# sosp2021/Reth

Measured on AMD Instinct MI355X. Metric: env-steps/sec + learner updates/sec, Ape-X DQN Pong, 1/2/4/8 MI355X, higher is better.
Workload: dtype f32

## Files before the change

### reth_amd/csrc/fc.hip

```cpp
#include <type_traits>
#include <utility>

#include "common.hpp"
#include "fc_rows.hpp"

namespace rth {

using f32x4 = __attribute__((ext_vector_type(4))) float;

constexpr int kFcTm = 64, kFcTn = 128, kFcThreads = 256;
__device__ __forceinline__ float fc_relu(float v) { return v < 0.0f ? 0.0f : v; }
constexpr int kFcBUnits = 8 * 3 * 64;

template <int... I, class F>
__device__ __forceinline__ void static_for(std::integer_sequence<int, I...>, F &&f) {
  (f(std::integral_constant<int, I>{}), ...);
}

template <int PF>
__global__ __launch_bounds__(kFcThreads) void k_fc_x9(const float *__restrict__ x, int64_t ldx, int M,
                                                      const float *__restrict__ w, int N, int K, int splits,
                                                      const float *__restrict__ bias, int relu,
                                                      float *__restrict__ out) {
  __shared__ uint4 bl[2][kFcBUnits];
  const int tid = threadIdx.x, lane = tid & 63, g = lane >> 4, r = lane & 15;
  const int wave = __builtin_amdgcn_readfirstlane(tid >> 6);
  const int tiles_n = N / kFcTn;
  const int tile = (int)blockIdx.x / splits, split = (int)blockIdx.x % splits;
  const int m0 = (tile / tiles_n) * kFcTm, n0 = (tile % tiles_n) * kFcTn;
  const int chunks = K / 32;
  const int c0 = chunks * split / splits, c1 = chunks * (split + 1) / splits;
  const int wn = tid & 127, wh = tid >> 7;
  const float *wrow = w + (int64_t)(n0 + wn) * K + 16 * wh;
  const float *xrow = x + (int64_t)(m0 + 16 * wave + r) * ldx + 8 * g;
  constexpr int NR = PF + 1;
  f32x4 wv[NR][4], xv[NR][2];
  auto load = [&](int c, f32x4 (&wl)[4], f32x4 (&xl)[2]) __attribute__((always_inline)) {
#pragma unroll
    for (int j = 0; j < 4; ++j) wl[j] = *reinterpret_cast<const f32x4 *>(wrow + 32 * c + 4 * j);
#pragma unroll
    for (int j = 0; j < 2; ++j) xl[j] = *reinterpret_cast<const f32x4 *>(xrow + 32 * c + 4 * j);
  };
  auto stage = [&](const f32x4 (&wl)[4], uint4 *buf) __attribute__((always_inline)) {
    const int nb = wn >> 4, rr = wn & 15;
#pragma unroll
    for (int h = 0; h < 2; ++h) {
      const float v[8] = {wl[2 * h][0], wl[2 * h][1], wl[2 * h][2], wl[2 * h][3],
                          wl[2 * h + 1][0], wl[2 * h + 1][1], wl[2 * h + 1][2], wl[2 * h + 1][3]};
      bf16x8 tr[3];
      split3_pk8(v, tr);
#pragma unroll
      for (int t = 0; t < 3; ++t) buf[(nb * 3 + t) * 64 + rr + 16 * (2 * wh + h)] = __builtin_bit_cast(uint4, tr[t]);
    }
  };
  f32x4 acc[8];
#pragma unroll
  for (int nb = 0; nb < 8; ++nb) acc[nb] = f32x4{0.f, 0.f, 0.f, 0.f};
  auto compute = [&](const f32x4 (&xl)[2], const uint4 *buf) __attribute__((always_inline)) {
    const float v[8] = {xl[0][0], xl[0][1], xl[0][2], xl[0][3], xl[1][0], xl[1][1], xl[1][2], xl[1][3]};
    bf16x8 af[3];
    split3_pk8(v, af);
#pragma unroll
    for (int nb = 0; nb < 8; ++nb) {
      bf16x8 b[3];
#pragma unroll
      for (int t = 0; t < 3; ++t) b[t] = __builtin_bit_cast(bf16x8, buf[(nb * 3 + t) * 64 + lane]);
      f32x4 a = acc[nb];
      a = __builtin_amdgcn_mfma_f32_16x16x32_bf16(af[2], b[2], a, 0, 0, 0);
      a = __builtin_amdgcn_mfma_f32_16x16x32_bf16(af[2], b[1], a, 0, 0, 0);
      a = __builtin_amdgcn_mfma_f32_16x16x32_bf16(af[1], b[2], a, 0, 0, 0);
      a = __builtin_amdgcn_mfma_f32_16x16x32_bf16(af[2], b[0], a, 0, 0, 0);
      a = __builtin_amdgcn_mfma_f32_16x16x32_bf16(af[1], b[1], a, 0, 0, 0);
      a = __builtin_amdgcn_mfma_f32_16x16x32_bf16(af[0], b[2], a, 0, 0, 0);
      a = __builtin_amdgcn_mfma_f32_16x16x32_bf16(af[1], b[0], a, 0, 0, 0);
      a = __builtin_amdgcn_mfma_f32_16x16x32_bf16(af[0], b[1], a, 0, 0, 0);
      a = __builtin_amdgcn_mfma_f32_16x16x32_bf16(af[0], b[0], a, 0, 0, 0);
      acc[nb] = a;
    }
  };
  auto iter = [&](int c, auto ic) __attribute__((always_inline)) {
    constexpr int i = decltype(ic)::value;
    constexpr int pr = i % NR, pl = i & 1;
    compute(xv[pr], bl[pl]);
    stage(wv[(i + 1) % NR], bl[pl ^ 1]);
    const int cn = c + NR < c1 ? c + NR : c1 - 1;
    load(cn, wv[pr], xv[pr]);
    __syncthreads();
  };
#pragma unroll
  for (int q = 0; q < NR; ++q) load(c0 + q < c1 ? c0 + q : c1 - 1, wv[q], xv[q]);
  stage(wv[0], bl[0]);
  __syncthreads();
  int c = c0;
  constexpr int U = 2 * NR;
  for (; c + U <= c1; c += U)
    static_for(std::make_integer_sequence<int, U>{}, [&](auto ic) __attribute__((always_inline)) {
      iter(c + decltype(ic)::value, ic);
    });
  static_for(std::make_integer_sequence<int, U>{}, [&](auto ic) __attribute__((always_inline)) {
    if (c + decltype(ic)::value < c1) iter(c + decltype(ic)::value, ic);
  });
  const int mrow = m0 + 16 * wave + 4 * g;
  if (splits == 1) {
#pragma unroll
    for (int nb = 0; nb < 8; ++nb) {
      const int n = n0 + 16 * nb + r;
      const float bn = bias ? bias[n] : 0.0f;
#pragma unroll
      for (int i = 0; i < 4; ++i) {
        const float v = radd(acc[nb][i], bn);
        out[(int64_t)(mrow + i) * N + n] = relu ? fc_relu(v) : v;
      }
    }
  } else {
    float *part = out + (int64_t)split * M * N;
#pragma unroll
    for (int nb = 0; nb < 8; ++nb)
#pragma unroll
      for (int i = 0; i < 4; ++i) part[(int64_t)(mrow + i) * N + n0 + 16 * nb + r] = acc[nb][i];
  }
}

constexpr int kFbTile = 128;
__host__ __device__ constexpr int fc_ta(int k) { return (int)((0x221210100ull >> (4 * (8 - k))) & 15); }
__host__ __device__ constexpr int fc_tb(int k) { return (int)((0x212012010ull >> (4 * (8 - k))) & 15); }
static_assert(fc_ta(0) == 2 && fc_tb(0) == 2 && fc_ta(3) == 2 && fc_tb(3) == 0 && fc_ta(5) == 0 && fc_tb(5) == 2 &&
                  fc_ta(8) == 0 && fc_tb(8) == 0 && fc_ta(6) == 1 && fc_tb(6) == 0,
              "term order");
constexpr int kFbUnits = 8 * 3 * 64;
template <int WAVES, int PF>
__global__ __launch_bounds__(WAVES * 64) void k_fc_x9t(const float *__restrict__ x, int64_t ldx, int M,
                                                      const float *__restrict__ w, int N, int K, int splits,
                                                      const float *__restrict__ bias, int relu,
                                                      float *__restrict__ out) {
  constexpr int T = WAVES * 64, WN = WAVES / 2, NB = 8 / WN;
  constexpr int RH = 2 * 2 * kFbTile / T;
  constexpr int NR = PF + 1;
  static_assert(WAVES == 4 || WAVES == 8, "4 or 8 waves");
  __shared__ uint4 sl[2][2][kFbUnits];
  const int tid = threadIdx.x, lane = tid & 63, g = lane >> 4, r = lane & 15;
  const int wave = __builtin_amdgcn_readfirstlane(tid >> 6), wm = wave & 1, wn = wave >> 1;
  const int tiles_n = N / kFbTile;
  const int tile = (int)blockIdx.x / splits, split = (int)blockIdx.x % splits;
  const int m0 = (tile / tiles_n) * kFbTile, n0 = (tile % tiles_n) * kFbTile;
  const int chunks = K / 32;
  const int c0 = chunks * split / splits, c1 = chunks * (split + 1) / splits;
  const float *src[RH];
#pragma unroll
  for (int j = 0; j < RH; ++j) {
    const int u = tid + j * T, op = u >> 8, rr = u & 127, h = (u >> 7) & 1;
    src[j] = op == 0 ? x + (int64_t)(m0 + rr) * ldx + 16 * h : w + (int64_t)(n0 + rr) * K + 16 * h;
  }
  f32x4 ring[NR][RH][4];
  auto load = [&](int c, f32x4 (&v)[RH][4]) __attribute__((always_inline)) {
#pragma unroll
    for (int j = 0; j < RH; ++j)
#pragma unroll
      for (int q = 0; q < 4; ++q) v[j][q] = *reinterpret_cast<const f32x4 *>(src[j] + 32 * c + 4 * q);
  };
  auto stage = [&](const f32x4 (&v)[RH][4], uint4 (*buf)[kFbUnits]) __attribute__((always_inline)) {
#pragma unroll
    for (int j = 0; j < RH; ++j) {
      const int u = tid + j * T, op = u >> 8, rr = u & 127, h = (u >> 7) & 1;
      const int blk = rr >> 4, rw = rr & 15;
#pragma unroll
      for (int hh = 0; hh < 2; ++hh) {
        const float vv[8] = {v[j][2 * hh][0], v[j][2 * hh][1], v[j][2 * hh][2], v[j][2 * hh][3],
                             v[j][2 * hh + 1][0], v[j][2 * hh + 1][1], v[j][2 * hh + 1][2], v[j][2 * hh + 1][3]};
        bf16x8 tr[3];
        split3_pk8(vv, tr);
#pragma unroll
        for (int t = 0; t < 3; ++t) buf[op][(blk * 3 + t) * 64 + rw + 16 * (2 * h + hh)] = __builtin_bit_cast(uint4, tr[t]);
      }
    }
  };
  f32x4 acc[4][NB];
#pragma unroll
  for (int mb = 0; mb < 4; ++mb)
#pragma unroll
    for (int nb = 0; nb < NB; ++nb) acc[mb][nb] = f32x4{0.f, 0.f, 0.f, 0.f};
  auto compute = [&](uint4 (*buf)[kFbUnits]) __attribute__((always_inline)) {
    bf16x8 af[4][3], bfr[NB][3];
#pragma unroll
    for (int mb = 0; mb < 4; ++mb)
#pragma unroll
      for (int t = 0; t < 3; ++t) af[mb][t] = __builtin_bit_cast(bf16x8, buf[0][((4 * wm + mb) * 3 + t) * 64 + lane]);
#pragma unroll
    for (int nb = 0; nb < NB; ++nb)
#pragma unroll
      for (int t = 0; t < 3; ++t)
        bfr[nb][t] = __builtin_bit_cast(bf16x8, buf[1][((NB * wn + nb) * 3 + t) * 64 + lane]);
#pragma unroll
    for (int k = 0; k < 9; ++k)
#pragma unroll
      for (int mb = 0; mb < 4; ++mb)
#pragma unroll
        for (int nb = 0; nb < NB; ++nb)
          acc[mb][nb] = __builtin_amdgcn_mfma_f32_16x16x32_bf16(af[mb][fc_ta(k)], bfr[nb][fc_tb(k)], acc[mb][nb], 0, 0, 0);
  };
  auto clampc = [&](int c) { return c < c1 ? c : c1 - 1; };
#pragma unroll
  for (int q = 0; q < NR; ++q) load(clampc(c0 + q), ring[q]);
  stage(ring[0], sl[0]);
  load(clampc(c0 + NR), ring[0]);
  __syncthreads();
  auto iter = [&](int i, auto ic) __attribute__((always_inline)) {
    constexpr int s = decltype(ic)::value;
    compute(sl[s & 1]);
    stage(ring[(s + 1) % NR], sl[(s + 1) & 1]);
    load(clampc(c0 + i + 1 + NR), ring[(s + 1) % NR]);
    __syncthreads();
  };
  const int n_it = c1 - c0;
  constexpr int U = 2 * NR;
  int i = 0;
  for (; i + U <= n_it; i += U)
    static_for(std::make_integer_sequence<int, U>{}, [&](auto ic) __attribute__((always_inline)) {
      iter(i + decltype(ic)::value, ic);
    });
  static_for(std::make_integer_sequence<int, U>{}, [&](auto ic) __attribute__((always_inline)) {
    if (i + decltype(ic)::value < n_it) iter(i + decltype(ic)::value, ic);
  });
  float *dst = splits == 1 ? out : out + (int64_t)split * M * N;
#pragma unroll
  for (int mb = 0; mb < 4; ++mb)
#pragma unroll
    for (int nb = 0; nb < NB; ++nb) {
      const int n = n0 + 16 * (NB * wn + nb) + r;
      const float bn = splits == 1 && bias ? bias[n] : 0.0f;
#pragma unroll
      for (int e = 0; e < 4; ++e) {
        const int m = m0 + 64 * wm + 16 * mb + 4 * g + e;
        float v = acc[mb][nb][e];
        if (splits == 1) {
          v = radd(v, bn);
          v = relu ? fc_relu(v) : v;
        }
        dst[(int64_t)m * N + n] = v;
      }
    }
}

constexpr int kFfTm = 64, kFfTn = 128, kFfThreads = 256;
template <int NST>
__global__ __launch_bounds__(kFfThreads) void k_fc_f32(const float *__restrict__ x, int64_t ldx, int M,
                                                       const float *__restrict__ w, int N, int K, int splits,
                                                       const float *__restrict__ bias, int relu,
                                                       float *__restrict__ out) {
  const int tid = threadIdx.x, lane = tid & 63, g = lane >> 4, r = lane & 15;
  const int wave = __builtin_amdgcn_readfirstlane(tid >> 6), wm = wave & 1, wn = wave >> 1;
  const int split = (int)blockIdx.x % splits, tile = (int)blockIdx.x / splits;
  const int tiles_n = N / kFfTn;
  const int m0 = (tile / tiles_n) * kFfTm + 32 * wm, n0 = (tile % tiles_n) * kFfTn + 64 * wn;
  const int chunks = K / 32;
  const int c0 = chunks * split / splits, c1 = chunks * (split + 1) / splits;
  const __amdgpu_buffer_rsrc_t xs = __builtin_amdgcn_make_buffer_rsrc(const_cast<float *>(x), 0,
                                                                      (int)(((int64_t)(M - 1) * ldx + K) * 4), 0x00020000);
  const __amdgpu_buffer_rsrc_t ws = __builtin_amdgcn_make_buffer_rsrc(const_cast<float *>(w), 0,
                                                                      (int)((int64_t)N * K * 4), 0x00020000);
  uint32_t xo[2], wo[4];
#pragma unroll
  for (int mb = 0; mb < 2; ++mb) {
    const int row = m0 + 16 * mb + r;
    xo[mb] = (uint32_t)(((int64_t)(row < M ? row : M - 1) * ldx + 8 * g) * 4);
  }
#pragma unroll
  for (int nb = 0; nb < 4; ++nb) wo[nb] = (uint32_t)(((int64_t)(n0 + 16 * nb + r) * K + 8 * g) * 4);
  f32x4 xa[NST][2][2], wb[NST][4][2];
  auto ld = [](__amdgpu_buffer_rsrc_t rs, uint32_t vo, int so) {
    return __builtin_bit_cast(f32x4, __builtin_amdgcn_raw_buffer_load_b128(rs, vo, so, 0));
  };
  auto load = [&](int c, f32x4 (&a)[2][2], f32x4 (&b)[4][2]) __attribute__((always_inline)) {
    const int so = c * 128;
#pragma unroll
    for (int nb = 0; nb < 4; ++nb)
#pragma unroll
      for (int h = 0; h < 2; ++h) b[nb][h] = ld(ws, wo[nb] + 16 * h, so);
#pragma unroll
    for (int mb = 0; mb < 2; ++mb)
#pragma unroll
      for (int h = 0; h < 2; ++h) a[mb][h] = ld(xs, xo[mb] + 16 * h, so);
  };
  f32x4 acc[2][4];
#pragma unroll
  for (int mb = 0; mb < 2; ++mb)
#pragma unroll
    for (int nb = 0; nb < 4; ++nb) acc[mb][nb] = f32x4{0.f, 0.f, 0.f, 0.f};
  auto compute = [&](const f32x4 (&a)[2][2], const f32x4 (&b)[4][2]) __attribute__((always_inline)) {
#pragma unroll
    for (int h = 0; h < 2; ++h)
#pragma unroll
      for (int t = 0; t < 4; ++t)
#pragma unroll
        for (int mb = 0; mb < 2; ++mb)
#pragma unroll
          for (int nb = 0; nb < 4; ++nb)
            acc[mb][nb] = __builtin_amdgcn_mfma_f32_16x16x4f32(a[mb][h][t], b[nb][h][t], acc[mb][nb], 0, 0, 0);
  };
#pragma unroll
  for (int s = 0; s < NST; ++s) load(c0 + s < c1 ? c0 + s : c1 - 1, xa[s], wb[s]);
  auto iter = [&](int c, auto is) __attribute__((always_inline)) {
    constexpr int s = decltype(is)::value;
    compute(xa[s], wb[s]);
    const int cn = c + NST < c1 ? c + NST : c1 - 1;
    load(cn, xa[s], wb[s]);
    __builtin_amdgcn_sched_barrier(0);
  };
  int c = c0;
  for (; c + NST <= c1; c += NST)
    static_for(std::make_integer_sequence<int, NST>{}, [&](auto is) __attribute__((always_inline)) {
      iter(c + decltype(is)::value, is);
    });
  static_for(std::make_integer_sequence<int, NST>{}, [&](auto is) __attribute__((always_inline)) {
    if (c + decltype(is)::value < c1) compute(xa[decltype(is)::value], wb[decltype(is)::value]);
  });
  float *dst = splits == 1 ? out : out + (int64_t)split * M * N;
#pragma unroll
  for (int mb = 0; mb < 2; ++mb)
#pragma unroll
    for (int i = 0; i < 4; ++i) {
      const int m = m0 + 16 * mb + 4 * g + i;
      if (m < M) {
#pragma unroll
        for (int nb = 0; nb < 4; ++nb) {
          const int n = n0 + 16 * nb + r;
          float v = acc[mb][nb][i];
          if (splits == 1) {
            v = radd(v, bias ? bias[n] : 0.0f);
            v = relu ? fc_relu(v) : v;
          }
          dst[(int64_t)m * N + n] = v;
        }
      }
    }
}

template <int MAXS>
__device__ __forceinline__ void fc_reduce_wg(int blk, const float *__restrict__ part, int splits, int64_t MN, int N,
                                             const float *__restrict__ bias, int relu, float *__restrict__ y,
                                             int64_t ldy) {
  const int64_t e4 = ((int64_t)blk * 256 + threadIdx.x) * 4;
  if (e4 >= MN) return;
  f32x4 v[MAXS];
#pragma unroll
  for (int k = 0; k < MAXS; ++k) v[k] = *reinterpret_cast<const f32x4 *>(part + (int64_t)(k < splits ? k : splits - 1) * MN + e4);
  f32x4 s = v[0];
#pragma unroll
  for (int k = 1; k < MAXS; ++k)
    if (k < splits) {
#pragma unroll
      for (int j = 0; j < 4; ++j) s[j] = radd(s[j], v[k][j]);
    }
  const int64_t m = e4 / N;
  const int n = (int)(e4 - m * N);
  f32x4 o;
#pragma unroll
  for (int j = 0; j < 4; ++j) {
    const float t = radd(s[j], bias ? bias[n + j] : 0.0f);
    o[j] = relu ? fc_relu(t) : t;
  }
  *reinterpret_cast<f32x4 *>(y + m * ldy + n) = o;
}

template <int MAXS>
__global__ __launch_bounds__(256) void k_fc_reduce(const float *__restrict__ part, int splits, int64_t MN, int N,
                                                   const float *__restrict__ bias, int relu, float *__restrict__ y,
                                                   int64_t ldy) {
  fc_reduce_wg<MAXS>((int)blockIdx.x, part, splits, MN, N, bias, relu, y, ldy);
}

constexpr int kRhRows = 4, kRhMaxN = 512;
template <int MAXS, int MAXA1>
__global__ __launch_bounds__(256) __attribute__((amdgpu_waves_per_eu(1, 3))) void k_fc_reduce_heads(const float *__restrict__ part, int splits, int M, int N,
                                                         const float *__restrict__ b1, int A,
                                                         const float *__restrict__ wa2, const float *__restrict__ wv2,
                                                         const float *__restrict__ ba2, const float *__restrict__ bv2,
                                                         float *__restrict__ heads, float *__restrict__ h1_out) {
  __shared__ f32x4 hs[kRhRows * kRhMaxN / 4];
  const int r0 = (int)blockIdx.x * kRhRows, N4 = N / 4;
  const int64_t MN = (int64_t)M * N;
  constexpr int PER = kRhRows * kRhMaxN / 4 / 256;
  f32x4 v[PER][MAXS];
  const __amdgpu_buffer_rsrc_t pr =
      __builtin_amdgcn_make_buffer_rsrc(const_cast<float *>(part), 0, (int)(splits * MN * 4), 0x00020000);
#pragma unroll
  for (int u = 0; u < PER; ++u) {
    const int i = (int)threadIdx.x + 256 * u, rr = i / N4;
    const int row = r0 + rr < M ? r0 + rr : M - 1;
    const uint32_t off = (uint32_t)(((int64_t)row * N + 4 * (i - rr * N4)) * 4);
#pragma unroll
    for (int k = 0; k < MAXS; ++k)
      v[u][k] = __builtin_bit_cast(
          f32x4, __builtin_amdgcn_raw_buffer_load_b128(pr, off, (int)((k < splits ? k : splits - 1) * MN * 4), 0));
  }
  __builtin_amdgcn_sched_barrier(0);
#pragma unroll
  for (int u = 0; u < PER; ++u) {
    const int i = (int)threadIdx.x + 256 * u, rr = i / N4, c = 4 * (i - rr * N4);
    if (i >= kRhRows * N4) break;
    f32x4 sum = v[u][0];
#pragma unroll
    for (int k = 1; k < MAXS; ++k)
      if (k < splits) {
#pragma unroll
        for (int j = 0; j < 4; ++j) sum[j] = radd(sum[j], v[u][k][j]);
      }
    f32x4 o;
#pragma unroll
    for (int j = 0; j < 4; ++j) o[j] = fc_relu(radd(sum[j], b1[c + j]));
    hs[i] = o;
    if (h1_out && r0 + rr < M) *reinterpret_cast<f32x4 *>(h1_out + (int64_t)(r0 + rr) * N + c) = o;
  }
  __syncthreads();
  if (threadIdx.x >= 16 * kRhRows) return;
  const int l = threadIdx.x & 15, rr = threadIdx.x >> 4;
  const int H = N / 2, cq = H / 64, A1 = A + 1;
  const f32x4 *ha = hs + rr * N4 + l * cq, *hv = hs + rr * N4 + H / 4 + l * cq;
  float acc[MAXA1];
#pragma unroll
  for (int a = 0; a < MAXA1; ++a) acc[a] = 0.0f;
#pragma unroll 1
  for (int k = 0; k < cq; ++k) {
    const f32x4 xa = ha[k], xv = hv[k];
    float4 w[MAXA1];
#pragma unroll
    for (int a = 0; a < MAXA1; ++a) {
      const int ac = a < A1 ? a : A;
      w[a] = reinterpret_cast<const float4 *>(ac < A ? wa2 + (int64_t)ac * H : wv2)[l * cq + k];
    }
#pragma unroll
    for (int a = 0; a < MAXA1; ++a)
      if (a < A1) {
        const f32x4 x = a < A ? xa : xv;
        const float4 ww = w[a];
        acc[a] = radd(radd(radd(radd(acc[a], rmul(x[0], ww.x)), rmul(x[1], ww.y)), rmul(x[2], ww.z)), rmul(x[3], ww.w));
      }
  }
#pragma unroll
  for (int a = 0; a < MAXA1; ++a)
#pragma unroll
    for (int o = 1; o < 16; o <<= 1) acc[a] = radd(acc[a], __shfl_xor(acc[a], o, 64));
  if (l == 0 && r0 + rr < M) {
    float *out = heads + (int64_t)(r0 + rr) * A1;
#pragma unroll
    for (int a = 0; a < MAXA1; ++a)
      if (a <= A) out[a] = radd(acc[a], a < A ? ba2[a] : bv2[0]);
  }
}

static_assert(kLrThreads == 256, "k_fc_reduce_rows runs k_linear_relu_rows' workgroups at 256 lanes");
template <int MAXS>
__global__ __launch_bounds__(256) void k_fc_reduce_rows(const float *__restrict__ part, int splits, int64_t MN, int N,
                                                        const float *__restrict__ bias, float *__restrict__ y,
                                                        int64_t ldy, int nred, const float *__restrict__ x,
                                                        int64_t ldx, int64_t r0, int64_t n_max,
                                                        const int64_t *__restrict__ n_dev,
                                                        const float *__restrict__ w, int K) {
  if ((int)blockIdx.x < nred)
    fc_reduce_wg<MAXS>((int)blockIdx.x, part, splits, MN, N, bias, 1, y, ldy);
  else
    linear_relu_rows_wg((int)blockIdx.x - nred, x, ldx, r0, n_max, n_dev, w, bias, K, N, y, ldy);
}

static const void *fc_reduce_fn(int splits, bool rows) {
  if (rows)
    return splits <= 4    ? reinterpret_cast<const void *>(&k_fc_reduce_rows<4>)
           : splits <= 8  ? reinterpret_cast<const void *>(&k_fc_reduce_rows<8>)
           : splits <= 16 ? reinterpret_cast<const void *>(&k_fc_reduce_rows<16>)
                          : reinterpret_cast<const void *>(&k_fc_reduce_rows<32>);
  return splits <= 4    ? reinterpret_cast<const void *>(&k_fc_reduce<4>)
         : splits <= 8  ? reinterpret_cast<const void *>(&k_fc_reduce<8>)
         : splits <= 16 ? reinterpret_cast<const void *>(&k_fc_reduce<16>)
                        : reinterpret_cast<const void *>(&k_fc_reduce<32>);
}
static int launch_fc_reduce(const float *part, int splits, int64_t MN, int N, const float *bias, int relu, float *y,
                            int64_t ldy, hipStream_t s) {
  RTH_REQUIRE(splits >= 1 && splits <= 32, "fc reduce: %d splits", splits);
  void *args[] = {&part, &splits, &MN, &N, &bias, &relu, &y, &ldy};
  RTH_HIP(hipLaunchKernel(fc_reduce_fn(splits, false), dim3((unsigned)((MN / 4 + 255) / 256)), dim3(256), args, 0, s));
  return RTH_OK;
}

static int fc_splits(int M, int N, int K) {
  const int tiles = (M / kFcTm) * (N / kFcTn), chunks = K / 32;
  int s = (256 + tiles - 1) / tiles;
  s = s < 1 ? 1 : (s > 32 ? 32 : s);
  return s < chunks ? s : chunks;
}

struct FcPlan {
  int big, splits;
};
constexpr int kFcMaxSplits = 16;
static FcPlan fc_plan(int M, int N, int K) {
  if (M % kFbTile || N % kFbTile) return FcPlan{0, fc_splits(M, N, K)};
  const int tiles = (M / kFbTile) * (N / kFbTile), chunks = K / 32;
  int s = (256 + tiles - 1) / tiles;
  s = s > kFcMaxSplits ? kFcMaxSplits : (s < 1 ? 1 : s);
  return FcPlan{1, s < chunks ? s : chunks};
}

static void fc_x9_launch(const FcPlan &p, const float *x, int64_t ldx, int M, const float *w, int N, int K,
                         const float *bias, int relu, float *out, hipStream_t s) {
  if (!p.big) {
    const int tiles = (M / kFcTm) * (N / kFcTn);
    hipLaunchKernelGGL(k_fc_x9<2>, dim3((unsigned)(tiles * p.splits)), dim3(kFcThreads), 0, s, x, ldx, M, w, N, K,
                       p.splits, bias, relu, out);
    return;
  }
  const dim3 grid((unsigned)((M / kFbTile) * (N / kFbTile) * p.splits));
  hipLaunchKernelGGL((k_fc_x9t<8, 1>), grid, dim3(512), 0, s, x, ldx, M, w, N, K, p.splits, bias, relu, out);
}

static int fcf_splits(int M, int N, int K) {
  const int tiles = ((M + kFfTm - 1) / kFfTm) * (N / kFfTn), chunks = K / 32;
  int s = 8;
  while (s > 1 && tiles * s > 512) s /= 2;
  return s < chunks ? s : chunks;
}

constexpr int kFwTn = 64, kFwThreads = 256;
constexpr int kFwAUnits = 8 * 3 * 64, kFwUnits = kFwAUnits + 4 * 3 * 64;
template <bool AT, int MB>
__device__ __forceinline__ void fc_bwd_tile(uint4 (*sl)[kFwUnits], const float *__restrict__ a, int64_t lda,
                                            const float *__restrict__ b, int64_t ldb, float *__restrict__ out,
                                            int64_t ldo, int m0, int n0, int c0, int c1) {
  constexpr int TM = 32 * MB, T = kFwThreads, NR = 2;
  constexpr int ATASKS = AT ? 4 * TM : 2 * TM, AJ = (ATASKS + T - 1) / T;
  const int tid = threadIdx.x, lane = tid & 63, g = lane >> 4, r = lane & 15;
  const int wave = __builtin_amdgcn_readfirstlane(tid >> 6), wm = wave & 1, wn = wave >> 1;
  const float *asrc[AJ];
#pragma unroll
  for (int j = 0; j < AJ; ++j) {
    const int u = tid + j * T, rr = u % TM, h = u / TM;
    asrc[j] = AT ? a + (int64_t)(8 * h) * lda + m0 + rr : a + (int64_t)(m0 + rr) * lda + 16 * h;
  }
  const float *bsrc = b + (int64_t)(8 * (tid >> 6)) * ldb + n0 + (tid & 63);
  f32x4 ra4[NR][AJ][4];
  float ra1[NR][AJ][8];
  float rb[NR][8];
  auto load = [&](int c, int s) __attribute__((always_inline)) {
#pragma unroll
    for (int j = 0; j < AJ; ++j)
      if (tid + j * T < ATASKS) {
        if constexpr (AT) {
#pragma unroll
          for (int q = 0; q < 8; ++q) ra1[s][j][q] = asrc[j][(int64_t)(32 * c + q) * lda];
        } else {
#pragma unroll
          for (int q = 0; q < 4; ++q) ra4[s][j][q] = *reinterpret_cast<const f32x4 *>(asrc[j] + 32 * c + 4 * q);
        }
      }
#pragma unroll
    for (int q = 0; q < 8; ++q) rb[s][q] = bsrc[(int64_t)(32 * c + q) * ldb];
  };
  auto put = [&](const float (&v)[8], uint4 *dst) __attribute__((always_inline)) {
    bf16x8 tr[3];
    split3_pk8(v, tr);
#pragma unroll
    for (int t = 0; t < 3; ++t) dst[t * 64] = __builtin_bit_cast(uint4, tr[t]);
  };
  auto stage = [&](int s, uint4 *buf) __attribute__((always_inline)) {
#pragma unroll
    for (int j = 0; j < AJ; ++j)
      if (tid + j * T < ATASKS) {
        const int u = tid + j * T, rr = u % TM, h = u / TM;
        uint4 *blk = buf + (rr >> 4) * 3 * 64 + (rr & 15);
        if constexpr (AT) {
          put(ra1[s][j], blk + 16 * h);
        } else {
#pragma unroll
          for (int hh = 0; hh < 2; ++hh) {
            const f32x4 lo = ra4[s][j][2 * hh], hi = ra4[s][j][2 * hh + 1];
            const float v[8] = {lo[0], lo[1], lo[2], lo[3], hi[0], hi[1], hi[2], hi[3]};
            put(v, blk + 16 * (2 * h + hh));
          }
        }
      }
    const int col = tid & 63;
    put(rb[s], buf + kFwAUnits + (col >> 4) * 3 * 64 + (col & 15) + 16 * (tid >> 6));
  };
  f32x4 acc[MB][2], lo[MB][2];
#pragma unroll
  for (int mb = 0; mb < MB; ++mb)
#pragma unroll
    for (int nb = 0; nb < 2; ++nb) acc[mb][nb] = lo[mb][nb] = f32x4{0.f, 0.f, 0.f, 0.f};
  auto compute = [&](const uint4 *buf) __attribute__((always_inline)) {
    bf16x8 af[MB][3], bfr[2][3];
#pragma unroll
    for (int mb = 0; mb < MB; ++mb)
#pragma unroll
      for (int t = 0; t < 3; ++t) af[mb][t] = __builtin_bit_cast(bf16x8, buf[((MB * wm + mb) * 3 + t) * 64 + lane]);
#pragma unroll
    for (int nb = 0; nb < 2; ++nb)
#pragma unroll
      for (int t = 0; t < 3; ++t)
        bfr[nb][t] = __builtin_bit_cast(bf16x8, buf[kFwAUnits + ((2 * wn + nb) * 3 + t) * 64 + lane]);
    static_assert(fc_ta(8) == 0 && fc_tb(8) == 0, "the leading term is the last");
#pragma unroll
    for (int k = 0; k < 9; ++k)
#pragma unroll
      for (int mb = 0; mb < MB; ++mb)
#pragma unroll
        for (int nb = 0; nb < 2; ++nb) {
          f32x4 &d = k < 8 ? lo[mb][nb] : acc[mb][nb];
          d = __builtin_amdgcn_mfma_f32_16x16x32_bf16(af[mb][fc_ta(k)], bfr[nb][fc_tb(k)], d, 0, 0, 0);
        }
  };
  auto clampc = [&](int c) { return c < c1 ? c : c1 - 1; };
  load(c0, 0);
  load(clampc(c0 + 1), 1);
  stage(0, sl[0]);
  load(clampc(c0 + 2), 0);
  __syncthreads();
  auto iter = [&](int i, auto is) __attribute__((always_inline)) {
    constexpr int s = decltype(is)::value;
    compute(sl[s]);
    stage(s ^ 1, sl[s ^ 1]);
    load(clampc(c0 + i + 3), s ^ 1);
    __syncthreads();
  };
  const int n_it = c1 - c0;
  int i = 0;
  for (; i + 2 <= n_it; i += 2) {
    iter(i, std::integral_constant<int, 0>{});
    iter(i + 1, std::integral_constant<int, 1>{});
  }
  if (i < n_it) iter(i, std::integral_constant<int, 0>{});
#pragma unroll
  for (int mb = 0; mb < MB; ++mb)
#pragma unroll
    for (int nb = 0; nb < 2; ++nb)
#pragma unroll
      for (int e = 0; e < 4; ++e)
        out[(int64_t)(m0 + 16 * (MB * wm + mb) + 4 * g + e) * ldo + n0 + 16 * (2 * wn + nb) + r] =
            radd(acc[mb][nb][e], lo[mb][nb][e]);
}

template <int MBD>
__global__ __launch_bounds__(kFwThreads) void k_fc_bwd(const float *__restrict__ gy, int64_t ldg,
                                                       const float *__restrict__ x, int64_t ldx,
                                                       const float *__restrict__ w, int B, int N, int K,
                                                       float *__restrict__ gx_out, float *__restrict__ gw_out,
                                                       int nblk_d, int sd, int sw) {
  __shared__ uint4 sl[2][kFwUnits];
  const int tiles_k = K / kFwTn;
  int blk = (int)blockIdx.x;
  if (blk < nblk_d) {
    const int tile = blk / sd, split = blk % sd, chunks = N / 32;
    fc_bwd_tile<false, MBD>(sl, gy, ldg, w, K, gx_out + (int64_t)split * B * K, K, (tile / tiles_k) * 32 * MBD,
                            (tile % tiles_k) * kFwTn, chunks * split / sd, chunks * (split + 1) / sd);
  } else {
    blk -= nblk_d;
    const int tile = blk / sw, split = blk % sw, chunks = B / 32;
    fc_bwd_tile<true, 4>(sl, gy, ldg, x, ldx, gw_out + (int64_t)split * N * K, K, (tile / tiles_k) * 128,
                         (tile % tiles_k) * kFwTn, chunks * split / sw, chunks * (split + 1) / sw);
  }
}

template <int MAXS>
__global__ __launch_bounds__(256) void k_fc_bwd_reduce(const float *__restrict__ pd, int sd, int64_t MNd,
                                                       float *__restrict__ gx, int nred_d,
                                                       const float *__restrict__ pw, int sw, int64_t MNw,
                                                       float *__restrict__ gw, int K) {
  if ((int)blockIdx.x < nred_d)
    fc_reduce_wg<MAXS>((int)blockIdx.x, pd, sd, MNd, K, nullptr, 0, gx, K);
  else
    fc_reduce_wg<MAXS>((int)blockIdx.x - nred_d, pw, sw, MNw, K, nullptr, 0, gw, K);
}

constexpr int kFwMaxSplits = 8;
struct FcBwdPlan {
  int mbd, tiles_d, sd, tiles_w, sw;
};
static FcBwdPlan fc_bwd_plan(int B, int N, int K) {
  auto splits = [](int tiles, int chunks) {
    int s = 1;
    while (2 * s * tiles <= 256 && 4 * s <= chunks && 2 * s <= kFwMaxSplits) s *= 2;
    return s;
  };
  FcBwdPlan p;
  p.mbd = B % 128 == 0 ? 4 : 2;
  p.tiles_d = (B / (32 * p.mbd)) * (K / kFwTn);
  p.sd = splits(p.tiles_d, N / 32);
  p.tiles_w = (N / 128) * (K / kFwTn);
  p.sw = splits(p.tiles_w, B / 32);
  return p;
}

}

using namespace rth;

extern "C" {

int rth_fc_bwd_supported(int64_t B, int64_t N, int64_t K) {
  return B > 0 && B % 64 == 0 && N > 0 && N % 128 == 0 && K > 0 && K % kFwTn == 0 && B * K < (1ll << 31) &&
                 N * K < (1ll << 31) && B * N < (1ll << 31)
             ? 1
             : 0;
}

int64_t rth_fc_bwd_workspace(int64_t B, int64_t N, int64_t K) {
  if (!rth_fc_bwd_supported(B, N, K)) return 0;
  const FcBwdPlan p = fc_bwd_plan((int)B, (int)N, (int)K);
  return (p.sd > 1 ? (int64_t)p.sd * B * K * 4 : 0) + (p.sw > 1 ? (int64_t)p.sw * N * K * 4 : 0);
}

int rth_fc_bwd(const float *gy, int64_t ldg, const float *x, int64_t ldx, const float *w, int64_t B, int64_t N,
               int64_t K, float *gx, float *gw, void *workspace, void *stream) {
  RTH_REQUIRE(gy && (gx || gw), "rth_fc_bwd: NULL gy, or neither gradient asked for");
  RTH_REQUIRE((!gx || w) && (!gw || x), "rth_fc_bwd: NULL operand of a gradient asked for");
  RTH_REQUIRE(rth_fc_bwd_supported(B, N, K), "rth_fc_bwd: shape %lld x %lld x %lld not built (B %% 64, N %% 128, K %% 64)",
              (long long)B, (long long)N, (long long)K);
  RTH_REQUIRE(ldg >= N && ldg % 4 == 0 && (!gw || (ldx >= K && ldx % 4 == 0)) && (B - 1) * ldg + N < (1ll << 31) &&
                  (!gw || (B - 1) * ldx + K < (1ll << 31)),
              "rth_fc_bwd: row strides %lld, %lld", (long long)ldg, (long long)ldx);
  RTH_REQUIRE(((reinterpret_cast<uintptr_t>(gy) | reinterpret_cast<uintptr_t>(x) | reinterpret_cast<uintptr_t>(w) |
                reinterpret_cast<uintptr_t>(gx) | reinterpret_cast<uintptr_t>(gw)) &
               15) == 0,
              "rth_fc_bwd: misaligned buffer");
  const FcBwdPlan p = fc_bwd_plan((int)B, (int)N, (int)K);
  const int sd = gx ? p.sd : 1, sw = gw ? p.sw : 1;
  RTH_REQUIRE((sd == 1 && sw == 1) || (workspace && (reinterpret_cast<uintptr_t>(workspace) & 15) == 0),
              "rth_fc_bwd: %d / %d splits need the workspace (rth_fc_bwd_workspace)", sd, sw);
  hipStream_t s = as_stream(stream);
  float *pd = static_cast<float *>(workspace);
  float *pw = pd ? pd + (p.sd > 1 ? (int64_t)p.sd * B * K : 0) : nullptr;
  float *od = sd > 1 ? pd : gx, *ow = sw > 1 ? pw : gw;
  const int nblk_d = gx ? p.tiles_d * sd : 0, nblk_w = gw ? p.tiles_w * sw : 0;
  const dim3 grid((unsigned)(nblk_d + nblk_w));
  if (p.mbd == 4)
    hipLaunchKernelGGL(k_fc_bwd<4>, grid, dim3(kFwThreads), 0, s, gy, ldg, x, ldx, w, (int)B, (int)N, (int)K, od, ow,
                       nblk_d, sd, sw);
  else
    hipLaunchKernelGGL(k_fc_bwd<2>, grid, dim3(kFwThreads), 0, s, gy, ldg, x, ldx, w, (int)B, (int)N, (int)K, od, ow,
                       nblk_d, sd, sw);
  RTH_LAUNCHED();
  if (sd > 1 || sw > 1) {
    const int64_t MNd = B * K, MNw = N * K;
    const int nred_d = sd > 1 ? (int)((MNd / 4 + 255) / 256) : 0, nred_w = sw > 1 ? (int)((MNw / 4 + 255) / 256) : 0;
    const dim3 rgrid((unsigned)(nred_d + nred_w));
    if (sd <= 4 && sw <= 4)
      hipLaunchKernelGGL(k_fc_bwd_reduce<4>, rgrid, dim3(256), 0, s, pd, sd, MNd, gx, nred_d, pw, sw, MNw, gw, (int)K);
    else
      hipLaunchKernelGGL(k_fc_bwd_reduce<8>, rgrid, dim3(256), 0, s, pd, sd, MNd, gx, nred_d, pw, sw, MNw, gw, (int)K);
    RTH_LAUNCHED();
  }
  return RTH_OK;
}

int rth_fc_x9_supported(int64_t M, int64_t N, int64_t K) {
  return M > 0 && M % kFcTm == 0 && N > 0 && N % kFcTn == 0 && K >= 32 && K % 32 == 0 && M * K < (1ll << 31) &&
                 N * K < (1ll << 31)
             ? 1
             : 0;
}

int64_t rth_fc_x9_workspace(int64_t M, int64_t N, int64_t K) {
  if (!rth_fc_x9_supported(M, N, K)) return 0;
  const int s = fc_plan((int)M, (int)N, (int)K).splits;
  return s > 1 ? (int64_t)s * M * N * 4 : 0;
}

int rth_fc_x9(const float *x, int64_t ldx, int64_t M, const float *w, int64_t N, int64_t K, const float *bias,
              int32_t relu, float *y, void *workspace, void *stream) {
  RTH_REQUIRE(x && w && y, "rth_fc_x9: NULL argument");
  RTH_REQUIRE(rth_fc_x9_supported(M, N, K), "rth_fc_x9: shape %lld x %lld x %lld not built (M %% 64, N %% 128, K %% 32)",
              (long long)M, (long long)N, (long long)K);
  RTH_REQUIRE(ldx >= K && ldx % 4 == 0, "rth_fc_x9: row stride %lld", (long long)ldx);
  RTH_REQUIRE(((reinterpret_cast<uintptr_t>(x) | reinterpret_cast<uintptr_t>(w) | reinterpret_cast<uintptr_t>(y)) &
               15) == 0,
              "rth_fc_x9: misaligned buffer");
  const FcPlan p = fc_plan((int)M, (int)N, (int)K);
  const int splits = p.splits;
  RTH_REQUIRE(splits == 1 || (workspace && (reinterpret_cast<uintptr_t>(workspace) & 15) == 0),
              "rth_fc_x9: %d splits need the workspace (rth_fc_x9_workspace)", splits);
  hipStream_t s = as_stream(stream);
  float *out = splits == 1 ? y : static_cast<float *>(workspace);
  fc_x9_launch(p, x, ldx, (int)M, w, (int)N, (int)K, bias, (int)relu, out, s);
  RTH_LAUNCHED();
  if (splits > 1) {
    const int64_t MN = M * N;
    const int rc = launch_fc_reduce(static_cast<const float *>(workspace), splits, MN, (int)N, bias, (int)relu, y, N, s);
    if (rc) return rc;
  }
  return RTH_OK;
}

int rth_fc_x9_rows_upto(const float *x, int64_t ldx, int64_t M, int64_t n_max, const int64_t *n_dev, const float *w,
                        int64_t N, int64_t K, const float *bias, float *y, void *workspace, void *stream) {
  RTH_REQUIRE(x && w && y && bias && n_dev, "rth_fc_x9_rows_upto: NULL argument");
  RTH_REQUIRE(rth_fc_x9_supported(M, N, K) && n_max >= M,
              "rth_fc_x9_rows_upto: shape %lld (+ %lld counted) x %lld x %lld not built (M %% 64, N %% 128, K %% 32)",
              (long long)M, (long long)(n_max - M), (long long)N, (long long)K);
  RTH_REQUIRE(ldx >= K && ldx % 4 == 0 &&
                  ((reinterpret_cast<uintptr_t>(x) | reinterpret_cast<uintptr_t>(w) | reinterpret_cast<uintptr_t>(y)) &
                   15) == 0,
              "rth_fc_x9_rows_upto: row stride %lld or misaligned buffer", (long long)ldx);
  const FcPlan p = fc_plan((int)M, (int)N, (int)K);
  const int splits = p.splits;
  if (splits == 1) {
    int rc = rth_fc_x9(x, ldx, M, w, N, K, bias, 1, y, workspace, stream);
    return rc ? rc : rth_linear_relu_rows_upto(x, ldx, M, n_max, n_dev, w, bias, K, N, y, N, stream);
  }
  RTH_REQUIRE(workspace && (reinterpret_cast<uintptr_t>(workspace) & 15) == 0,
              "rth_fc_x9_rows_upto: %d splits need the workspace (rth_fc_x9_workspace)", splits);
  hipStream_t s = as_stream(stream);
  float *part = static_cast<float *>(workspace);
  fc_x9_launch(p, x, ldx, (int)M, w, (int)N, (int)K, bias, 1, part, s);
  RTH_LAUNCHED();
  const int64_t MN = M * N;
  const int nred = (int)((MN / 4 + 255) / 256), nrows = n_max > M ? (int)((N + kLrCols - 1) / kLrCols) : 0;
  RTH_REQUIRE(splits <= 32, "rth_fc_x9_rows_upto: %d splits", splits);
  {
    const float *cpart = part;
    int Ni = (int)N, Ki = (int)K;
    int64_t ldy = N, r0 = M;
    void *args[] = {&cpart, const_cast<int *>(&splits), const_cast<int64_t *>(&MN), &Ni, &bias, &y, &ldy,
                    const_cast<int *>(&nred), &x, &ldx, &r0, &n_max, &n_dev, &w, &Ki};
    RTH_HIP(hipLaunchKernel(fc_reduce_fn(splits, true), dim3((unsigned)(nred + nrows)), dim3(256), args, 0, s));
  }
  return RTH_OK;
}

int rth_fc1_heads_supported(int64_t M, int64_t N, int64_t K, int32_t A) {
  if (!rth_fc_x9_supported(M, N, K) || N > kRhMaxN || N % 128 || A < 1 || A + 1 > 8) return 0;
  const int s = fc_plan((int)M, (int)N, (int)K).splits;
  return s >= 2 && s <= 16 ? 1 : 0;
}

int rth_fc1_heads(const float *x, int64_t ldx, int64_t M, const float *w1, int64_t N, int64_t K, const float *b1,
                  int32_t A, const float *const *fc2_params, float *heads, float *h1_out, void *workspace,
                  void *stream) {
  RTH_REQUIRE(x && w1 && b1 && fc2_params && heads && workspace, "rth_fc1_heads: NULL argument");
  RTH_REQUIRE(rth_fc1_heads_supported(M, N, K, A), "rth_fc1_heads: shape %lld x %lld x %lld, A %d not built",
              (long long)M, (long long)N, (long long)K, A);
  RTH_REQUIRE((int64_t)fc_plan((int)M, (int)N, (int)K).splits * M * N * 4 < ((int64_t)1 << 31),
              "rth_fc1_heads: split-K partials past 2 GiB");
  for (int i = 0; i < 4; ++i) RTH_REQUIRE(fc2_params[i], "rth_fc1_heads: NULL FC2 parameter %d", i);
  RTH_REQUIRE(ldx >= K && ldx % 4 == 0 &&
                  ((reinterpret_cast<uintptr_t>(x) | reinterpret_cast<uintptr_t>(w1) |
                    reinterpret_cast<uintptr_t>(workspace) | reinterpret_cast<uintptr_t>(h1_out)) &
                   15) == 0,
              "rth_fc1_heads: row stride %lld or misaligned buffer", (long long)ldx);
  const FcPlan p = fc_plan((int)M, (int)N, (int)K);
  hipStream_t s = as_stream(stream);
  float *part = static_cast<float *>(workspace);
  fc_x9_launch(p, x, ldx, (int)M, w1, (int)N, (int)K, b1, 1, part, s);
  RTH_LAUNCHED();
  const dim3 grid((unsigned)((M + kRhRows - 1) / kRhRows));
  if (p.splits <= 8)
    hipLaunchKernelGGL((k_fc_reduce_heads<8, 8>), grid, dim3(256), 0, s, part, p.splits, (int)M, (int)N, b1, (int)A,
                       fc2_params[0], fc2_params[1], fc2_params[2], fc2_params[3], heads, h1_out);
  else
    hipLaunchKernelGGL((k_fc_reduce_heads<16, 8>), grid, dim3(256), 0, s, part, p.splits, (int)M, (int)N, b1, (int)A,
                       fc2_params[0], fc2_params[1], fc2_params[2], fc2_params[3], heads, h1_out);
  RTH_LAUNCHED();
  return RTH_OK;
}

int rth_fc_f32_supported(int64_t M, int64_t N, int64_t K) {
  return M > 0 && N > 0 && N % kFfTn == 0 && K >= 32 && K % 32 == 0 && M * K < (1ll << 31) && N * K < (1ll << 31) &&
                 M * N * 32 < (1ll << 31)
             ? 1
             : 0;
}

int64_t rth_fc_f32_workspace(int64_t M, int64_t N, int64_t K) {
  if (!rth_fc_f32_supported(M, N, K)) return 0;
  const int s = fcf_splits((int)M, (int)N, (int)K);
  return s > 1 ? (int64_t)s * M * N * 4 : 0;
}

int rth_fc_f32(const float *x, int64_t ldx, int64_t M, const float *w, int64_t N, int64_t K, const float *bias,
               int32_t relu, float *y, void *workspace, void *stream) {
  RTH_REQUIRE(x && w && y, "rth_fc_f32: NULL argument");
  RTH_REQUIRE(rth_fc_f32_supported(M, N, K), "rth_fc_f32: shape %lld x %lld x %lld not built (N %% 128, K %% 32)",
              (long long)M, (long long)N, (long long)K);
  RTH_REQUIRE(ldx >= K && ldx % 4 == 0 && ((M - 1) * ldx + K) * 4 < (1ll << 31), "rth_fc_f32: row stride %lld",
              (long long)ldx);
  RTH_REQUIRE(((reinterpret_cast<uintptr_t>(x) | reinterpret_cast<uintptr_t>(w) | reinterpret_cast<uintptr_t>(y)) &
               15) == 0,
              "rth_fc_f32: misaligned buffer");
  const int splits = fcf_splits((int)M, (int)N, (int)K);
  RTH_REQUIRE(splits == 1 || (workspace && (reinterpret_cast<uintptr_t>(workspace) & 15) == 0),
              "rth_fc_f32: %d splits need the workspace (rth_fc_f32_workspace)", splits);
  hipStream_t s = as_stream(stream);
  const int tiles = (int)((M + kFfTm - 1) / kFfTm) * (int)(N / kFfTn);
  float *out = splits == 1 ? y : static_cast<float *>(workspace);
  const void *fn = reinterpret_cast<const void *>(&k_fc_f32<3>);
  int Mi = (int)M, Ni = (int)N, Ki = (int)K, re = (int)relu;
  void *args[] = {&x, &ldx, &Mi, &w, &Ni, &Ki, const_cast<int *>(&splits), &bias, &re, &out};
  RTH_HIP(hipLaunchKernel(fn, dim3((unsigned)(tiles * splits)), dim3(kFfThreads), args, 0, s));
  if (splits > 1) {
    const int64_t MN = M * N;
    const int rc = launch_fc_reduce(static_cast<const float *>(workspace), splits, MN, (int)N, bias, (int)relu, y, N, s);
    if (rc) return rc;
  }
  return RTH_OK;
}

}
```

Baseline: 510,200.

## Ping-pong wave halves between MFMA compute and load/stage in big FC kernel

Specializes the 8-wave FC GEMM kernel so the two halves of the block alternate phases: one half runs MFMA compute while the other stages the split-bf16 operands into LDS and issues global loads, with an extra barrier per iteration separating the halves. Loads are remapped so each half owns one operand (x or w), and LDS fragment reads are reordered. The aim is to overlap matrix-core work with memory and conversion work inside a block, at the cost of twice as many barriers and a fixed 8-wave configuration.

Result: no change. 514,800, median of 6 (+0.9%).

```diff
diff --git a/reth_amd/csrc/fc.hip b/reth_amd/csrc/fc.hip
--- a/reth_amd/csrc/fc.hip
+++ b/reth_amd/csrc/fc.hip
@@ -121,57 +121,48 @@
   }
 }
 
-constexpr int kFbTile = 128;
+constexpr int kFbTile = 128, kFbThreads = 512;
 __host__ __device__ constexpr int fc_ta(int k) { return (int)((0x221210100ull >> (4 * (8 - k))) & 15); }
 __host__ __device__ constexpr int fc_tb(int k) { return (int)((0x212012010ull >> (4 * (8 - k))) & 15); }
 static_assert(fc_ta(0) == 2 && fc_tb(0) == 2 && fc_ta(3) == 2 && fc_tb(3) == 0 && fc_ta(5) == 0 && fc_tb(5) == 2 &&
                   fc_ta(8) == 0 && fc_tb(8) == 0 && fc_ta(6) == 1 && fc_tb(6) == 0,
               "term order");
 constexpr int kFbUnits = 8 * 3 * 64;
-template <int WAVES, int PF>
-__global__ __launch_bounds__(WAVES * 64) void k_fc_x9t(const float *__restrict__ x, int64_t ldx, int M,
-                                                      const float *__restrict__ w, int N, int K, int splits,
-                                                      const float *__restrict__ bias, int relu,
-                                                      float *__restrict__ out) {
-  constexpr int T = WAVES * 64, WN = WAVES / 2, NB = 8 / WN;
-  constexpr int RH = 2 * 2 * kFbTile / T;
-  constexpr int NR = PF + 1;
-  static_assert(WAVES == 4 || WAVES == 8, "4 or 8 waves");
+__global__ __launch_bounds__(kFbThreads) void k_fc_x9t(const float *__restrict__ x, int64_t ldx, int M,
+                                                       const float *__restrict__ w, int N, int K, int splits,
+                                                       const float *__restrict__ bias, int relu,
+                                                       float *__restrict__ out) {
+  constexpr int NB = 2;
+  constexpr int NR = 2;
   __shared__ uint4 sl[2][2][kFbUnits];
   const int tid = threadIdx.x, lane = tid & 63, g = lane >> 4, r = lane & 15;
   const int wave = __builtin_amdgcn_readfirstlane(tid >> 6), wm = wave & 1, wn = wave >> 1;
+  const int half = wave >> 2;
   const int tiles_n = N / kFbTile;
   const int tile = (int)blockIdx.x / splits, split = (int)blockIdx.x % splits;
   const int m0 = (tile / tiles_n) * kFbTile, n0 = (tile % tiles_n) * kFbTile;
   const int chunks = K / 32;
   const int c0 = chunks * split / splits, c1 = chunks * (split + 1) / splits;
-  const float *src[RH];
-#pragma unroll
-  for (int j = 0; j < RH; ++j) {
-    const int u = tid + j * T, op = u >> 8, rr = u & 127, h = (u >> 7) & 1;
-    src[j] = op == 0 ? x + (int64_t)(m0 + rr) * ldx + 16 * h : w + (int64_t)(n0 + rr) * K + 16 * h;
-  }
-  f32x4 ring[NR][RH][4];
-  auto load = [&](int c, f32x4 (&v)[RH][4]) __attribute__((always_inline)) {
-#pragma unroll
-    for (int j = 0; j < RH; ++j)
-#pragma unroll
-      for (int q = 0; q < 4; ++q) v[j][q] = *reinterpret_cast<const f32x4 *>(src[j] + 32 * c + 4 * q);
-  };
-  auto stage = [&](const f32x4 (&v)[RH][4], uint4 (*buf)[kFbUnits]) __attribute__((always_inline)) {
-#pragma unroll
-    for (int j = 0; j < RH; ++j) {
-      const int u = tid + j * T, op = u >> 8, rr = u & 127, h = (u >> 7) & 1;
-      const int blk = rr >> 4, rw = rr & 15;
-#pragma unroll
-      for (int hh = 0; hh < 2; ++hh) {
-        const float vv[8] = {v[j][2 * hh][0], v[j][2 * hh][1], v[j][2 * hh][2], v[j][2 * hh][3],
-                             v[j][2 * hh + 1][0], v[j][2 * hh + 1][1], v[j][2 * hh + 1][2], v[j][2 * hh + 1][3]};
-        bf16x8 tr[3];
-        split3_pk8(vv, tr);
-#pragma unroll
-        for (int t = 0; t < 3; ++t) buf[op][(blk * 3 + t) * 64 + rw + 16 * (2 * h + hh)] = __builtin_bit_cast(uint4, tr[t]);
-      }
+  const int64_t sld = half == 0 ? ldx : (int64_t)K;
+  const float *src = (half == 0 ? x + (int64_t)m0 * ldx : w + (int64_t)n0 * K) +
+                     (int64_t)(32 * (wave & 3) + (lane >> 2)) * sld + 8 * (lane & 3);
+  f32x4 ring[NR][4];
+  auto load = [&](int c, f32x4 (&v)[4]) __attribute__((always_inline)) {
+#pragma unroll
+    for (int j = 0; j < 2; ++j)
+#pragma unroll
+      for (int q = 0; q < 2; ++q) v[2 * j + q] = *reinterpret_cast<const f32x4 *>(src + 16 * j * sld + 32 * c + 4 * q);
+  };
+  auto stage = [&](const f32x4 (&v)[4], uint4 (*buf)[kFbUnits]) __attribute__((always_inline)) {
+    uint4 *dst = buf[half] + 2 * (wave & 3) * 3 * 64 + (lane >> 2) + 16 * (lane & 3);
+#pragma unroll
+    for (int j = 0; j < 2; ++j) {
+      const float vv[8] = {v[2 * j][0], v[2 * j][1], v[2 * j][2], v[2 * j][3],
+                           v[2 * j + 1][0], v[2 * j + 1][1], v[2 * j + 1][2], v[2 * j + 1][3]};
+      bf16x8 tr[3];
+      split3_pk8(vv, tr);
+#pragma unroll
+      for (int t = 0; t < 3; ++t) dst[(3 * j + t) * 64] = __builtin_bit_cast(uint4, tr[t]);
     }
   };
   f32x4 acc[4][NB];
@@ -181,15 +172,15 @@
     for (int nb = 0; nb < NB; ++nb) acc[mb][nb] = f32x4{0.f, 0.f, 0.f, 0.f};
   auto compute = [&](uint4 (*buf)[kFbUnits]) __attribute__((always_inline)) {
     bf16x8 af[4][3], bfr[NB][3];
-#pragma unroll
-    for (int mb = 0; mb < 4; ++mb)
-#pragma unroll
-      for (int t = 0; t < 3; ++t) af[mb][t] = __builtin_bit_cast(bf16x8, buf[0][((4 * wm + mb) * 3 + t) * 64 + lane]);
-#pragma unroll
-    for (int nb = 0; nb < NB; ++nb)
-#pragma unroll
-      for (int t = 0; t < 3; ++t)
-        bfr[nb][t] = __builtin_bit_cast(bf16x8, buf[1][((NB * wn + nb) * 3 + t) * 64 + lane]);
+    auto read_a = [&](int t) __attribute__((always_inline)) {
+#pragma unroll
+      for (int mb = 0; mb < 4; ++mb) af[mb][t] = __builtin_bit_cast(bf16x8, buf[0][((4 * wm + mb) * 3 + t) * 64 + lane]);
+    };
+    auto read_b = [&](int t) __attribute__((always_inline)) {
+#pragma unroll
+      for (int nb = 0; nb < NB; ++nb) bfr[nb][t] = __builtin_bit_cast(bf16x8, buf[1][((NB * wn + nb) * 3 + t) * 64 + lane]);
+    };
+    read_a(2), read_b(2), read_b(1), read_a(1), read_b(0), read_a(0);
 #pragma unroll
     for (int k = 0; k < 9; ++k)
 #pragma unroll
@@ -204,23 +195,40 @@
   stage(ring[0], sl[0]);
   load(clampc(c0 + NR), ring[0]);
   __syncthreads();
-  auto iter = [&](int i, auto ic) __attribute__((always_inline)) {
-    constexpr int s = decltype(ic)::value;
-    compute(sl[s & 1]);
-    stage(ring[(s + 1) % NR], sl[(s + 1) & 1]);
-    load(clampc(c0 + i + 1 + NR), ring[(s + 1) % NR]);
-    __syncthreads();
-  };
   const int n_it = c1 - c0;
-  constexpr int U = 2 * NR;
-  int i = 0;
-  for (; i + U <= n_it; i += U)
+  auto run = [&](auto mf) __attribute__((always_inline)) {
+    constexpr bool MF = decltype(mf)::value;
+    auto half_step_end = [&]() __attribute__((always_inline)) {
+      __builtin_amdgcn_sched_barrier(0);
+      __syncthreads();
+      __builtin_amdgcn_sched_barrier(0);
+    };
+    auto refill = [&](int i, auto ic) __attribute__((always_inline)) {
+      constexpr int s = decltype(ic)::value;
+      stage(ring[(s + 1) % NR], sl[(s + 1) & 1]);
+      load(clampc(c0 + i + 1 + NR), ring[(s + 1) % NR]);
+    };
+    auto iter = [&](int i, auto ic) __attribute__((always_inline)) {
+      constexpr int s = decltype(ic)::value;
+      if constexpr (MF) compute(sl[s & 1]);
+      else refill(i, ic);
+      half_step_end();
+      if constexpr (MF) refill(i, ic);
+      else compute(sl[s & 1]);
+      half_step_end();
+    };
+    constexpr int U = 2 * NR;
+    int i = 0;
+    for (; i + U <= n_it; i += U)
+      static_for(std::make_integer_sequence<int, U>{}, [&](auto ic) __attribute__((always_inline)) {
+        iter(i + decltype(ic)::value, ic);
+      });
     static_for(std::make_integer_sequence<int, U>{}, [&](auto ic) __attribute__((always_inline)) {
-      iter(i + decltype(ic)::value, ic);
+      if (i + decltype(ic)::value < n_it) iter(i + decltype(ic)::value, ic);
     });
-  static_for(std::make_integer_sequence<int, U>{}, [&](auto ic) __attribute__((always_inline)) {
-    if (i + decltype(ic)::value < n_it) iter(i + decltype(ic)::value, ic);
-  });
+  };
+  if (half == 0) run(std::true_type{});
+  else run(std::false_type{});
   float *dst = splits == 1 ? out : out + (int64_t)split * M * N;
 #pragma unroll
   for (int mb = 0; mb < 4; ++mb)
@@ -509,7 +517,7 @@
     return;
   }
   const dim3 grid((unsigned)((M / kFbTile) * (N / kFbTile) * p.splits));
-  hipLaunchKernelGGL((k_fc_x9t<8, 1>), grid, dim3(512), 0, s, x, ldx, M, w, N, K, p.splits, bias, relu, out);
+  hipLaunchKernelGGL(k_fc_x9t, grid, dim3(kFbThreads), 0, s, x, ldx, M, w, N, K, p.splits, bias, relu, out);
 }
 
 static int fcf_splits(int M, int N, int K) {
```
